# lzzcd001/MeshDiffusion

Measured on AMD Instinct MI355X. Metric: denoise steps/sec on 64^3x4 DMTet grids (sample-steps/s = n_gpus*batch*steps/wall), higher is better.
Workload: dtype f16f6 in the Winograd convs behind a GroupNorm (fp16 hi*hi MFMA + MX block-scaled e2m3 cross terms in a K-concatenated scaled MFMA at twice the e4m3 rate; operands and weights equalised per input channel by a power of two: md_wino_equaliser, after the load-time calibration from the measured operand

## Files before the change

### include/meshdiffusion_hip.h

```cpp
#ifndef MESHDIFFUSION_HIP_H
#define MESHDIFFUSION_HIP_H

#include <stdint.h>

#ifdef __cplusplus
extern "C" {
#endif

#define MD_OK 0
#define MD_ERR_BAD_ARG (-1)
#define MD_ERR_UNSUPPORTED (-2)
#define MD_ERR_NO_DEVICE (-3)

#define MD_ABI_VERSION 16

enum {
  MD_CFG_C3_128 = 0,
  MD_CFG_C3_128_K16 = 1,
  MD_CFG_C3_32 = 2,
  MD_CFG_C3_LOW = 3,
  MD_CFG_C3_S2 = 4,
  MD_CFG_G1_128 = 5,
  MD_CFG_G1_128_LOW = 6,
  MD_CFG_G1_64_LOW = 7,
// ... 26 lines not shown
  float alpha;
  int32_t cfg;
  int32_t batch;
  int32_t rows;
  int32_t rows_alloc;
  int32_t kdim;
  int32_t D, H, W;
  int32_t ups;
  int32_t a_src;
  int32_t out_mode;
  int32_t a_rows;
  int64_t a_bstride;
  int64_t bias_bstride;
  int64_t res_bstride;
  int64_t b_bstride;
  float* partial;
  int32_t ksplit;
  int32_t prec;
  double* stats;
  int32_t stagger;
  int32_t b_mode;
  const void* b2;
  const float* b_ac;
  int64_t b2_bstride;
  int32_t b_split;
  int32_t b_silu;
} MdGemmConvArgs;

int md_abi_version(void);
int md_device_count(void);

int md_gemm_conv(const MdGemmConvArgs* args, void* stream);
int64_t md_gemm_conv_partial_bytes(const MdGemmConvArgs* args);
int md_gemm_conv_cfg_info(int32_t cfg, int32_t* nt, int32_t* kc, int32_t* cols,
                          int32_t* taps, int32_t* lds_bytes, int32_t* threads);

int md_pack_weights(const float* w, void* wpk, int32_t rows, int32_t kdim, int32_t taps,
                    int64_t s_row, int64_t s_k, int64_t s_tap, int32_t nt, int32_t kc,
                    int32_t prec, void* stream);
int64_t md_packed_weight_bytes(int32_t rows, int32_t kdim, int32_t taps, int32_t nt, int32_t kc);

int md_gn_stats(const float* x, double* sums, int32_t batch, int32_t C, int64_t P,
                int32_t c_total, int32_t c_off, void* stream);
int md_gn_finalize(const double* sums, const float* gamma, const float* beta,
                   float* params, int32_t batch, int32_t c_total, int32_t groups,
                   int64_t P, float eps, float* ac, void* stream);
int md_gn_apply(const float* x, const float* params, void* out, void* out_raw, int32_t batch,
                int32_t C, int64_t P, int32_t c_total, int32_t c_off, int32_t norm,
                int32_t silu, float drop_p, uint64_t drop_seed, void* stream);
int md_dropout_scale(float* out, int32_t batch, int32_t C, int64_t P, int32_t c_total, int32_t c_off,
                     float drop_p, uint64_t drop_seed, void* stream);
int md_zero(void* p, int64_t bytes, void* stream);

int md_timestep_embedding(const float* t, float* emb, int32_t batch, int32_t dim, void* stream);
int md_linear(const float* x, const float* w, const float* bias, float* y, int32_t batch,
              int32_t in_dim, int32_t out_dim, int32_t silu_in, void* stream);

int md_fold_dx(const float* y, const float* bias, float* out, int32_t batch, int32_t co, int32_t kx, int32_t rows_alloc,
               int32_t D, int32_t H, int32_t W, void* stream);
int md_ncdhw_to_s16b_xfold(const float* x, void* out, int32_t batch, int32_t C, int32_t kx, int32_t c_pad, int32_t D, int32_t H,
                           int32_t W, void* stream);
int md_ncdhw_to_s16b(const float* x, void* out, int32_t batch, int32_t C, int32_t c_pad,
                     int64_t P, void* stream);
int md_f32b_to_ncdhw(const float* x, float* out, int32_t batch, int32_t C, int64_t P, void* stream);
int md_ncdhw_to_f32b(const float* x, float* out, int32_t batch, int32_t C, int64_t P, void* stream);
int md_s16b_to_ncdhw(const void* x, float* out, int32_t batch, int32_t C, int64_t P, void* stream);
// ... 257 lines not shown
```

### meshdiffusion_amd/_lib.py

```python
import ctypes as C
import os

_HERE = os.path.dirname(os.path.abspath(__file__))
LIB_PATH = os.environ.get("MD_LIB") or os.path.join(_HERE, "libmeshdiffusion_hip.so")

(CFG_C3_128, CFG_C3_128_K16, CFG_C3_32, CFG_C3_LOW, CFG_C3_S2, CFG_G1_128, CFG_G1_128_LOW, CFG_G1_64_LOW,
 CFG_C3_128_V2, CFG_C3_128_SW, CFG_C3_128_PIPE) = range(11)
(CFG_C3_128_FAST, CFG_C5_128_K16, CFG_C5_32_K16, CFG_C3_128_W4, CFG_C3X_32, CFG_C5X_32_K16, CFG_C3X_128_K16, CFG_C5X_128,
 CFG_G1_128_N128) = range(14, 23)
OUT_F32B, OUT_S16B, OUT_NCDHW = 0, 1, 2
PREC_BF16X3, PREC_FP16X2 = 0, 1
A_PACKED, A_S16B = 0, 1
B_S16B, B_F32B_GN = 0, 1
CORRECTOR_LANGEVIN, CORRECTOR_ALD = 0, 1
SDE_REVERSE_DIFFUSION, SDE_EULER_MARUYAMA = 0, 1
LANGEVIN_SLABS = 64

CFG_NT_KC = {
    CFG_C3_128: (128, 32), CFG_C3_128_K16: (128, 16), CFG_C3_32: (32, 32), CFG_C3_LOW: (128, 32),
    CFG_C3_S2: (128, 32), CFG_G1_128: (128, 32), CFG_G1_128_LOW: (128, 32), CFG_G1_64_LOW: (64, 32),
    CFG_C3_128_V2: (128, 32), CFG_C3_128_SW: (128, 32), CFG_C3_128_PIPE: (128, 32),
    CFG_C3_128_FAST: (128, 32), CFG_C5_128_K16: (128, 16), CFG_C5_32_K16: (32, 16), CFG_C3_128_W4: (128, 32), CFG_C3X_32: (32, 32), CFG_C5X_32_K16: (32, 16), CFG_C3X_128_K16: (128, 16), CFG_C5X_128: (128, 32), CFG_G1_128_N128: (128, 32),
}
ABLATION_CFG_NT_KC = {c: (128, 32) for c in (101, 102, 103, 104, 105, 111, 113, 114, 116, 117, 118, 122)}


class MdGemmConvArgs(C.Structure):
    _fields_ = [
        ("a", C.c_void_p), ("b", C.c_void_p), ("out", C.c_void_p), ("bias", C.c_void_p),
        ("residual", C.c_void_p), ("alpha", C.c_float), ("cfg", C.c_int32), ("batch", C.c_int32),
        ("rows", C.c_int32), ("rows_alloc", C.c_int32), ("kdim", C.c_int32), ("D", C.c_int32),
        ("H", C.c_int32), ("W", C.c_int32), ("ups", C.c_int32), ("a_src", C.c_int32),
        ("out_mode", C.c_int32), ("a_rows", C.c_int32), ("a_bstride", C.c_int64),
        ("bias_bstride", C.c_int64), ("res_bstride", C.c_int64), ("b_bstride", C.c_int64), ("partial", C.c_void_p), ("ksplit", C.c_int32), ("prec", C.c_int32),
        ("stats", C.c_void_p), ("stagger", C.c_int32), ("b_mode", C.c_int32), ("b2", C.c_void_p), ("b_ac", C.c_void_p),
        ("b2_bstride", C.c_int64), ("b_split", C.c_int32), ("b_silu", C.c_int32),
    ]


class MdPackJob(C.Structure):
    _fields_ = [
        ("w", C.c_void_p), ("out", C.c_void_p), ("s_row", C.c_int64), ("s_k", C.c_int64), ("s_tap", C.c_int64),
        ("n_items", C.c_int64), ("block0", C.c_int64), ("rows", C.c_int32), ("kdim", C.c_int32), ("taps", C.c_int32),
        ("nt", C.c_int32), ("kc", C.c_int32), ("prec", C.c_int32), ("flip", C.c_int32), ("kind", C.c_int32),
    ]


PACK_WPK, PACK_WINO, PACK_WINO_F6 = 0, 1, 2
WINO_FMT = {False: 0, "f8": 1, "f6": 2}
ABI_VERSION = 16
_P, _I32, _I64, _F, _U64 = C.c_void_p, C.c_int32, C.c_int64, C.c_float, C.c_uint64

SIGNATURES = {
    "md_abi_version": (C.c_int, []),
    "md_device_count": (C.c_int, []),
    "md_gemm_conv": (C.c_int, [C.POINTER(MdGemmConvArgs), _P]),
    "md_gemm_conv_partial_bytes": (_I64, [C.POINTER(MdGemmConvArgs)]),
    "md_gemm_conv_cfg_info": (C.c_int, [_I32] + [C.POINTER(C.c_int32)] * 6),
    "md_pack_weights": (C.c_int, [_P, _P, _I32, _I32, _I32, _I64, _I64, _I64, _I32, _I32, _I32, _P]),
    "md_packed_weight_bytes": (_I64, [_I32, _I32, _I32, _I32, _I32]),
    "md_gn_stats": (C.c_int, [_P, _P, _I32, _I32, _I64, _I32, _I32, _P]),
    "md_gn_finalize": (C.c_int, [_P, _P, _P, _P, _I32, _I32, _I32, _I64, _F, _P, _P]),
    "md_gn_apply": (C.c_int, [_P, _P, _P, _P, _I32, _I32, _I64, _I32, _I32, _I32, _I32, _F, _U64, _P]),
    "md_dropout_scale": (C.c_int, [_P, _I32, _I32, _I64, _I32, _I32, _F, _U64, _P]),
    "md_zero": (C.c_int, [_P, _I64, _P]),
    "md_timestep_embedding": (C.c_int, [_P, _P, _I32, _I32, _P]),
    "md_linear": (C.c_int, [_P, _P, _P, _P, _I32, _I32, _I32, _I32, _P]),
    "md_ncdhw_to_s16b_xfold": (C.c_int, [_P, _P, _I32, _I32, _I32, _I32, _I32, _I32, _I32, _P]),
    "md_fold_dx": (C.c_int, [_P, _P, _P, _I32, _I32, _I32, _I32, _I32, _I32, _I32, _P]),
    "md_ncdhw_to_s16b": (C.c_int, [_P, _P, _I32, _I32, _I32, _I64, _P]),
    "md_f32b_to_ncdhw": (C.c_int, [_P, _P, _I32, _I32, _I64, _P]),
    "md_ncdhw_to_f32b": (C.c_int, [_P, _P, _I32, _I32, _I64, _P]),
    "md_s16b_to_ncdhw": (C.c_int, [_P, _P, _I32, _I32, _I64, _P]),
    "md_nin_f32": (C.c_int, [_P, _P, _I32, _I32, _P, _P, _P, _I32, _I32, _I64, _I32, _P]),
    "md_wino_operand_bytes": (_I64, [_I32, _I32, _I32, _I32, _I32]),
    "md_wino_prep": (C.c_int, [_P, _P, _I32, _I32, _P, _I32, _I32, _P, _I32, _I32, _I32, _I32, _F, _U64, _P]),
    "md_wino_weight_bytes": (_I64, [_I32, _I32]),
    "md_wino_pack_weights": (C.c_int, [_P, _P, _I32, _I32, _I64, _I64, _I32, _P]),
    "md_conv3_wino": (C.c_int, [_P, _P, _P, _P, _I64, _P, _I64, _P, _I32, _I32, _I32, _I32, _I32, _I32, _I32, _P]),
    "md_wino_equaliser": (C.c_int, [_P, _P, _P, _I32, _I32, _I64, _I64, _P, _P]),
    "md_wino_equaliser_measured": (C.c_int, [_P, _P, _P, _P, _I32, _I32, _I64, _I64, _P, _P]),
    "md_wino_operand_ms": (C.c_int, [_P, _P, _I32, _I32, _P, _I32, _I32, _I64, _P, _P]),
    "md_wino_prep_f8": (C.c_int, [_P, _P, _I32, _I32, _P, _I32, _I32, _P, _P, _I32, _I32, _I32, _I32, _P]),
    "md_wino_weight_bytes_f8": (_I64, [_I32, _I32]),
    "md_wino_pack_weights_f8": (C.c_int, [_P, _P, _P, _I32, _I32, _I64, _I64, _P]),
    "md_conv3_wino_f8": (C.c_int, [_P, _P, _P, _P, _I64, _P, _I64, _P, _I32, _I32, _I32, _I32, _I32, _I32, _P]),
    "md_absmax": (C.c_int, [_P, _I64, _P, _P]),
    "md_wino_prep_dual_f6": (C.c_int, [_P, _I32, _P, _P, _P, _F, _P, _I32, _I32, _I32, _I32, _P]),
    "md_conv3_wino_f6_scaled": (C.c_int, [_P, _P, _P, _P, _I64, _P, _I64, _P, _I32, _I32, _I32, _I32, _I32, _I32, _F, _P, _P]),
    "md_wino_prep_f6": (C.c_int, [_P, _P, _I32, _I32, _P, _I32, _I32, _P, _P, _I32, _I32, _I32, _I32, _P]),
# ... 139 lines not shown
```

### meshdiffusion_amd/build.py

```python
import os
import shutil
import subprocess
import sys

HERE = os.path.dirname(os.path.abspath(__file__))
CSRC = os.path.join(HERE, "csrc")
INCLUDE = os.path.join(os.path.dirname(HERE), "include")
_SUFFIX = os.environ.get("MD_LIB_SUFFIX", "")
OBJDIR = os.path.join(CSRC, "build" + _SUFFIX)
LIB_PATH = os.path.join(HERE, f"libmeshdiffusion_hip{_SUFFIX}.so")
ARCH = "gfx950"
SOURCES = ["capi.hip", "gemm_conv.hip", "conv3_main.hip", "conv3_wino.hip", "conv3_s2.hip", "conv3_head.hip", "conv3_stem.hip", "pack_batch.hip", "wino_prep2.hip", "wino_eq.hip", "norm.hip", "elementwise.hip", "sde_steps.hip", "attention.hip", "nin_stream.hip", "block_pass.hip", "train.hip", "backward.hip", "wgrad.hip", "wgrad_wino.hip", "dmtet.hip", "dmtet_bwd.hip", "pointcloud.hip", "raster.hip", "antialias.hip", "interp.hip", "fixedtopo.hip", "visibility.hip"]
FLAGS = ["-O3", "-std=c++17", "-fPIC", f"--offload-arch={ARCH}", f"-I{INCLUDE}", f"-I{CSRC}",
         "-munsafe-fp-atomics", "-Wno-unused-result"]


def _hipcc():
    exe = shutil.which("hipcc") or "/opt/rocm/bin/hipcc"
    if not os.path.exists(exe):
        raise RuntimeError("hipcc not found: cannot build libmeshdiffusion_hip.so")
    return exe


def _newer(target, deps):
    if not os.path.exists(target):
        return True
    t = os.path.getmtime(target)
    return any(os.path.getmtime(d) > t for d in deps)


def build(verbose=False, force=False):
    from concurrent.futures import ThreadPoolExecutor
    hipcc = _hipcc()
    os.makedirs(OBJDIR, exist_ok=True)
    headers = [os.path.join(CSRC, "md_common.h"), os.path.join(CSRC, "md_pack.h"), os.path.join(CSRC, "md_prep_f6.h"), os.path.join(CSRC, "md_raster_snap.h"), os.path.join(CSRC, "md_gather.h"), os.path.join(INCLUDE, "meshdiffusion_hip.h")]
    flags = FLAGS + (["-DMD_BUILD_ABLATIONS"] if os.environ.get("MD_BUILD_ABLATIONS") == "1" else [])
    flags = flags + os.environ.get("MD_EXTRA_DEFINES", "").split()
    stamp = os.path.join(OBJDIR, "flags.txt")
    if not os.path.exists(stamp) or open(stamp).read() != " ".join(flags):
        force = True
    objs, jobs = [], []
    for src in SOURCES:
        sp = os.path.join(CSRC, src)
        if not os.path.exists(sp):
            raise RuntimeError(f"missing source {sp}")
# ... 27 lines not shown
```

### meshdiffusion_amd/hip_ops.py

```python
import ctypes as C
import math
import os

import torch

from . import _lib
from ._lib import (A_PACKED, A_S16B, PREC_BF16X3, PREC_FP16X2, CFG_C3_128, CFG_C3_128_V2, CFG_C3_128_SW, CFG_C3_128_PIPE, CFG_C3_128_FAST, CFG_C5_128_K16, CFG_C5_32_K16, CFG_C3_128_W4, CFG_C3X_32, CFG_C5X_32_K16, CFG_C3X_128_K16, CFG_C5X_128, CFG_G1_128_N128, CFG_C3_128_K16, CFG_C3_32, CFG_C3_LOW, CFG_C3_S2,
                   CFG_G1_128, CFG_G1_128_LOW, CFG_G1_64_LOW, CFG_NT_KC, OUT_F32B, OUT_NCDHW, OUT_S16B,
                   MdGemmConvArgs, check)


CFG_ABL1, CFG_ABL2, CFG_ABL3, CFG_ABL4, CFG_ABL5 = 101, 102, 103, 104, 105
CFG_F1, CFG_F3, CFG_F4, CFG_F6, CFG_F7, CFG_F8 = 111, 113, 114, 116, 117, 118
CFG_FAST_EC = 122
CONV_STAGGER = int(os.environ.get("MD_CONV_STAGGER", "0"))
DEBUG_ACT_FP16 = 2 if os.environ.get("MD_DEBUG_ACT_FP16") == "1" else 0
_MODES = ("bf16x3", "fp16x2", "f16f8", "f16f6")
DEFAULT_PRECISION = os.environ.get("MD_PRECISION", "bf16x3")
FORCE_PRECISION = os.environ.get("MD_FORCE_PRECISION")
WINO_EQ = os.environ.get("MD_WINO_EQ", "1") == "1"
F8_RAW = os.environ.get("MD_F8_RAW", "0") == "1"


def _decode(mode):
# ... 236 lines not shown

def prewarm_packs():
    layers = list(_PACK_LAYERS)
    _PACK_LAYERS.clear()
    n = 0
    for layer in layers:
        used = layer.__dict__.pop("_md_used", None) or {}
        if not PACK_BATCH:
            continue
        cache = layer.__dict__.get("_md_cache") or {}
        for name, (params, builder) in used.items():
            old = cache.get(name)
            consumed = old is not None and getattr(old[1], "_data", None) is not None
            obj = layer._cached(name, params, builder, mark=False)
            if consumed and hasattr(obj, "request"):
                obj.request()
                n += 1
    flush_packs()
    return n


def pack_s16b_from_matrix(w_kp, device):
    lib = _lib.load()
    w = w_kp.detach().to(device=device, dtype=torch.float32).contiguous()
    K, P = w.shape
    out = s16b_empty(1, K, P, device)
    check(lib.md_ncdhw_to_s16b(_ptr(w), _ptr(out), 1, K, K, P, _stream()), "md_ncdhw_to_s16b")
    return out


def gemm_conv(*, cfg, a, b, out, batch, rows, rows_alloc, kdim, dims, bias=None, bias_bstride=0,
              residual=None, res_bstride=0, alpha=1.0, ups=0, a_src=A_PACKED, a_rows=0, a_bstride=0,
              b_bstride=None, out_mode=OUT_F32B, ksplit=1, prec=PREC_BF16X3, stats=None, stagger=None,
              b_f32=None):
    lib = _lib.load()
    D, H, W = dims
    args = MdGemmConvArgs()
    args.a, args.out = a.data_ptr(), out.data_ptr()
    if b_f32 is not None:
        parts = b_f32["parts"]
        assert 1 <= len(parts) <= 2 and sum(c for _, c in parts) == kdim and all(c % 8 == 0 for _, c in parts)
        pin = D * H * W // (8 if ups else 1)
        args.b, args.b_split = parts[0][0].data_ptr(), parts[0][1]
        b_bstride = parts[0][1] * pin
        if len(parts) == 2:
            args.b2, args.b2_bstride = parts[1][0].data_ptr(), parts[1][1] * pin
        ac = b_f32.get("ac")
        args.b_ac = ac.data_ptr() if ac is not None else None
        args.b_silu = 1 if b_f32.get("silu") else 0
        args.b_mode = _lib.B_F32B_GN
    else:
        args.b = b.data_ptr()
    args.bias = bias.data_ptr() if bias is not None else None
    args.residual = residual.data_ptr() if residual is not None else None
    args.alpha = alpha
    args.cfg, args.batch, args.rows, args.rows_alloc, args.kdim = cfg, batch, rows, rows_alloc, kdim
    args.D, args.H, args.W, args.ups = D, H, W, ups
    args.a_src, args.out_mode, args.a_rows = a_src, out_mode, a_rows
    args.a_bstride, args.bias_bstride, args.res_bstride = a_bstride, bias_bstride, res_bstride
    if b_bstride is None:
        pin = D * H * W
        if ups:
            pin //= 8
        elif cfg == CFG_C3_S2:
            pin *= 8
        b_bstride = (kdim // 8) * 2 * pin * 8
    args.b_bstride = b_bstride
    args.prec = prec
    args.stats = stats.data_ptr() if stats is not None else None
    args.stagger = CONV_STAGGER if stagger is None else int(stagger)
    part = None
    if ksplit > 1:
        if out_mode != OUT_F32B:
            raise ValueError("split-K supports F32B output only")
        args.ksplit = ksplit
        part = torch.empty((ksplit * batch * rows_alloc * D * H * W,), dtype=torch.float32, device=out.device)
        args.partial = part.data_ptr()
    if PROFILE is None:
        check(lib.md_gemm_conv(C.byref(args), _stream()), f"md_gemm_conv(cfg={cfg})")
    else:
        taps = _lib.cfg_info(cfg)["taps"]
        flops = 2.0 * batch * rows * kdim * taps * D * H * W
        pin = D * H * W // (8 if ups else 1) * (8 if cfg == CFG_C3_S2 else 1)
        abytes = 4.0 * (batch * kdim * pin + rows * kdim * taps + batch * rows * D * H * W * (2 if residual is not None else 1))
        e0, e1 = torch.cuda.Event(enable_timing=True), torch.cuda.Event(enable_timing=True)
        e0.record()
        check(lib.md_gemm_conv(C.byref(args), _stream()), f"md_gemm_conv(cfg={cfg})")
        e1.record()
        PROFILE.append((cfg, flops, e0, e1, abytes,
                        f"{kdim}->{rows}@{D}x{H}x{W}" + ("/ups" if ups else "") + (f"/ks{ksplit}" if ksplit > 1 else "") +
                        ("/res" if residual is not None else "") + ("/stats" if stats is not None else "")))
    return out


WINO = os.environ.get("MD_WINO", "1") == "1"
WINO_PREP_V2 = os.environ.get("MD_WINO_PREP_V2", "1") == "1"
WINO_TRAIN_FWD = os.environ.get("MD_WINO_TRAIN_FWD", "1") == "1"


class WinoWeight:

    def __init__(self, w, device, kind="conv"):
        lib = _lib.load()
        w = w.detach().to(device=device, dtype=torch.float32).contiguous()
        _require_cuda(w, "weight")
        assert w.dim() == 5 and tuple(w.shape[2:]) == (3, 3, 3)
        if kind == "conv":
            self.rows, self.kdim = w.shape[0], w.shape[1]
            s_row, s_k, flip = self.kdim * 27, 27, 0
        elif kind == "conv_dgrad":
            self.rows, self.kdim = w.shape[1], w.shape[0]
            s_row, s_k, flip = 27, self.rows * 27, 1
        else:
            raise ValueError(kind)
        nbytes = lib.md_wino_weight_bytes(self.rows, self.kdim)
        if nbytes <= 0:
            raise _lib.MeshDiffusionHipError("md_wino_weight_bytes: unsupported weight shape")
        self._data, self._queued = None, False
        self._src = dict(kind=_lib.PACK_WINO, w=w, w_off=0, nbytes=nbytes, rows=self.rows, kdim=self.kdim, taps=9, s_row=s_row,
                         s_k=s_k, s_tap=0, nt=0, kc=0, prec=PREC_BF16X3, flip=flip)

    def request(self):
# ... 670 lines not shown
    check(lib.md_ddim_step(_ptr(x64), _ptr(eps), _ptr(mask), _ptr(coef), _ptr(partial), _ptr(pmask), int(ch), _ptr(x_out),
                           _ptr(x0_out), _ptr(x_f32), B, Cc, P, _stream()), "md_ddim_step")
    return x_out, x0_out, x_f32


def inpaint_blend_(x, src, pmask, gmask, ch, src_bstride=0):
    lib = _lib.load()
    B, Cc = x.shape[0], x.shape[1]
    P = x[0, 0].numel()
    check(lib.md_inpaint_blend(_ptr(x), _ptr(src), _ptr(pmask), _ptr(gmask), B, Cc, ch, P, src_bstride,
                               _stream()), "md_inpaint_blend")
    return x


def inpaint_renoise_(x, x_mean, z, pmask, gmask, coef, ch):
    lib = _lib.load()
    B, Cc = x.shape[0], x.shape[1]
    P = x[0, 0].numel()
    check(lib.md_inpaint_renoise(_ptr(x), _ptr(x_mean), _ptr(z), _ptr(pmask), _ptr(gmask), _ptr(coef), B, Cc,
                                 ch, P, _stream()), "md_inpaint_renoise")
    return x


def ksplit_for(cfg, batch, rows, kdim, spatial_out):
    info = _lib.cfg_info(cfg)
    tiles = max(1, spatial_out ** 3 // info["cols"]) * batch * ((rows + info["nt"] - 1) // info["nt"])
    ncc = kdim // info["kc"]
    ks = 1
    while tiles * ks < 256 and ks * 2 <= ncc and ks < 32:
        ks *= 2
    return ks


def conv_cfg_for(spatial, stride=1):
    if stride == 2:
        return CFG_C3_S2
    return CFG_C3_128_FAST if spatial % 8 == 0 else CFG_C3_LOW


NIN_N128 = os.environ.get("MD_NIN_N128", "1") == "1"


def gemm_cfg_for(ncols, nrows, hbm_bound=False):
    if hbm_bound and NIN_N128 and ncols % 128 == 0 and ncols >= 32768:
        return CFG_G1_128_N128
    if ncols % 256 == 0:
        return CFG_G1_128
    return CFG_G1_128_LOW if nrows % 128 == 0 else CFG_G1_64_LOW


def attn_scale(channels):
    return float(int(channels) ** (-0.5))


__all__ = [n for n in dir() if not n.startswith("_")]
_ = math
```

### meshdiffusion_amd/lib/diffusion/models/layers.py

```python
import math

import numpy as np
import torch
import torch.nn as nn

from .... import hip_ops as ops


def variance_scaling(scale, mode, distribution, in_axis=1, out_axis=0, dtype=torch.float32, device="cpu"):
    def init(shape, dtype=dtype, device=device):
        receptive = np.prod(shape) / shape[in_axis] / shape[out_axis]
        fan_in, fan_out = shape[in_axis] * receptive, shape[out_axis] * receptive
        denom = {"fan_in": fan_in, "fan_out": fan_out, "fan_avg": (fan_in + fan_out) / 2}[mode]
        var = scale / denom
        if distribution == "normal":
            return torch.randn(*shape, dtype=dtype, device=device) * np.sqrt(var)
        if distribution == "uniform":
            return (torch.rand(*shape, dtype=dtype, device=device) * 2.0 - 1.0) * np.sqrt(3 * var)
        raise ValueError("invalid distribution for variance scaling initializer")

    return init


def default_init(scale=1.0):
# ... 117 lines not shown
        f8 = (not b_f32.get("wino_only")) and ops.wino_f8_ok(
            S_out, drop=b_f32.get("drop"), keep=bool(b_f32.get("keep")), parts=b_f32["parts"],
            normalised=b_f32.get("ac") is not None
            or (ops.WINO_EQ and hasattr(wino, "measured") and wino.measured() is not None))
        if f8 and owner is not None and wino.site in getattr(owner, "md_bf16x3_sites", ()):
            f8 = False
        compact = (not b_f32.get("wino_only")) and ops.prep_compact_ok(ups, S_out, S_out, S_out, drop=b_f32.get("drop"), keep=bool(b_f32.get("keep")))
        nin = b_f32.get("nin")
        if (nin is not None and f8 == "f6" and not compact and not ups and not b_f32.get("drop") and not b_f32.get("keep")
                and not b_f32.get("wino_only") and ops.block_pass_ok(b_f32["parts"], nin[0].rows, B, S_out, S_out, S_out)):
            t, b_f32["res_out"] = ops.wino_prep_nin(b_f32["parts"], b_f32.get("ac"), b_f32.get("silu"), B, S_out,
                                                    wino.eq() if hasattr(wino, "eq") else None, nin[0], nin[1])
        else:
            t = ops.wino_prep(b_f32["parts"], b_f32.get("ac"), b_f32.get("silu"), ups, B, S_out, drop=b_f32.get("drop"),
                              keep=bool(b_f32.get("keep")), f8=f8, eq=wino.eq() if f8 and hasattr(wino, "eq") else None, compact=compact)
        if b_f32.get("keep"):
            b_f32["t_out"] = t
        ops.conv3_wino(wino(f8) if f8 else wino(), t, B, S_out, bias=bias, bias_bstride=bias_bstride, residual=residual,
                       res_bstride=res_bstride or 0, stats=stats, out=out)
        if f8 and ops.AUDIT is not None:
            t3 = ops.wino_prep(b_f32["parts"], b_f32.get("ac"), b_f32.get("silu"), ups, B, S_out, compact=compact)
            ref = ops.conv3_wino(wino(), t3, B, S_out, bias=bias, bias_bstride=bias_bstride, residual=residual, res_bstride=res_bstride or 0)
            ops.AUDIT.append(dict(owner=getattr(wino, "owner", None), site=getattr(wino, "site", None), fmt=f8, cin=pw.kdim, cout=pw.rows,
                                  S=S_out, rel_l2=float((torch.linalg.vector_norm(out - ref, dtype=torch.float64)
                                                         / torch.linalg.vector_norm(ref, dtype=torch.float64).clamp_min(1e-300)).item())))
            del t3, ref
        if stats is not None:
            out._md_sums = stats
        elif hasattr(out, "_md_sums"):
            del out._md_sums
        return out
    if b_f32 is not None and b_f32.get("wino_only"):
        b_f32 = None
    ksplit = ops.ksplit_for(pw.cfg, B, pw.rows, pw.kdim, S_out) if out_mode == ops.OUT_F32B else 1
    stats = None
    if (want_stats and ops.FUSE_GN_STATS and ((pw.cfg == ops.CFG_C3_128_FAST and ksplit == 1)
                                              or (ksplit > 1 and ops.SPLITK_STATS and P <= 512 and B * rows_alloc >= 2048))
            and out_mode == ops.OUT_F32B and rows_alloc == pw.rows):
        stats = ops.stats_zeros(B, rows_alloc, dev)
    ops.gemm_conv(cfg=pw.cfg, a=pw.data, b=act_s16, out=out, batch=B, rows=pw.rows,
                  rows_alloc=rows_alloc, kdim=pw.kdim, dims=(S_out, S_out, S_out), bias=bias,
                  bias_bstride=bias_bstride, residual=residual, res_bstride=res_bstride or 0, ups=ups,
                  out_mode=out_mode, ksplit=ksplit, prec=pw.prec, stats=stats, b_f32=b_f32)
    if stats is not None:
        out._md_sums = stats
    elif hasattr(out, "_md_sums"):
        del out._md_sums
    return out


def run_gemm(pw, act_s16, B, P, *, bias=None, bias_bstride=0, residual=None, out=None, out_mode=ops.OUT_F32B,
             alpha=1.0, b_bstride=None, b_f32=None):
    rows_alloc = ((pw.rows + 7) // 8) * 8
    dev = act_s16.device if act_s16 is not None else b_f32["parts"][0][0].device
    if out is None:
        out = (ops.f32b_empty if out_mode == ops.OUT_F32B else ops.s16b_empty)(B, rows_alloc, P, dev)
    return ops.gemm_conv(cfg=pw.cfg, a=pw.data, b=act_s16, out=out, batch=B, rows=pw.rows,
                         rows_alloc=rows_alloc, kdim=pw.kdim, dims=(1, 1, P), bias=bias,
                         bias_bstride=bias_bstride, residual=residual,
                         res_bstride=rows_alloc * P if residual is not None else 0, alpha=alpha,
                         out_mode=out_mode, b_bstride=b_bstride, b_f32=b_f32)


class NIN(HipLayer):

    def __init__(self, in_dim, num_units, init_scale=0.1):
        super().__init__()
        self.W = nn.Parameter(default_init(scale=init_scale)((in_dim, num_units)), requires_grad=True)
        self.b = nn.Parameter(torch.zeros(num_units), requires_grad=True)

    def packed(self, P, hbm_bound=False):
        rows = self.W.shape[1]
        cfg = ops.gemm_cfg_for(P, rows, hbm_bound)
        return self._cached(f"w{cfg}", [self.W], lambda: ops.PackedWeight(self.W, "nin", cfg, self.W.device))

    def forward_s16(self, act_s16, B, P, residual=None, out_mode=ops.OUT_F32B):
        return run_gemm(self.packed(P), act_s16, B, P, bias=self.b, residual=residual, out_mode=out_mode)

    def forward(self, x):
        parts, B, P, spatial = _parts_of(x)
        act = ops.gn_apply(parts, None, B, P, norm=False, silu=False)
        return ops.f32b_to_ncdhw(self.forward_s16(act, B, P), spatial)


class AttnBlock(HipLayer):

    def __init__(self, channels):
        super().__init__()
        self.GroupNorm_0 = nn.GroupNorm(num_groups=32, num_channels=channels, eps=1e-6)
        self.NIN_0 = NIN(channels, channels)
        self.NIN_1 = NIN(channels, channels)
        self.NIN_2 = NIN(channels, channels)
        self.NIN_3 = NIN(channels, channels, init_scale=0.0)
        self.channels = channels
# ... 278 lines not shown
```

Baseline: 114.1.

## Add split-K small-spatial conv kernel for low-resolution 3x3x3 and NIN layers

Adds a new HIP kernel for convolutions and 1x1 GEMMs at tiny spatial sizes (4^3 and 8^3). It stages the whole halo in LDS, double-buffers weights and activations, and splits the K dimension across many workgroups, targeting roughly 256 groups in total. It also adds a finishing kernel that reduces the split-K partials and computes the GroupNorm statistics in the same pass. The aim is to fill the GPU on low-resolution layers that the existing configs launch with too few tiles, at the cost of extra partial-buffer traffic and a reduction pass.

```diff
diff --git a/include/meshdiffusion_hip.h b/include/meshdiffusion_hip.h
--- a/include/meshdiffusion_hip.h
+++ b/include/meshdiffusion_hip.h
@@ -82,6 +82,7 @@
 
 int md_gemm_conv(const MdGemmConvArgs* args, void* stream);
 int64_t md_gemm_conv_partial_bytes(const MdGemmConvArgs* args);
+int md_small_conv(const MdGemmConvArgs* args, int32_t taps, void* stream);
 int md_gemm_conv_cfg_info(int32_t cfg, int32_t* nt, int32_t* kc, int32_t* cols,
                           int32_t* taps, int32_t* lds_bytes, int32_t* threads);
 
diff --git a/meshdiffusion_amd/_lib.py b/meshdiffusion_amd/_lib.py
--- a/meshdiffusion_amd/_lib.py
+++ b/meshdiffusion_amd/_lib.py
@@ -56,6 +56,7 @@
     "md_device_count": (C.c_int, []),
     "md_gemm_conv": (C.c_int, [C.POINTER(MdGemmConvArgs), _P]),
     "md_gemm_conv_partial_bytes": (_I64, [C.POINTER(MdGemmConvArgs)]),
+    "md_small_conv": (C.c_int, [C.POINTER(MdGemmConvArgs), _I32, _P]),
     "md_gemm_conv_cfg_info": (C.c_int, [_I32] + [C.POINTER(C.c_int32)] * 6),
     "md_pack_weights": (C.c_int, [_P, _P, _I32, _I32, _I32, _I64, _I64, _I64, _I32, _I32, _I32, _P]),
     "md_packed_weight_bytes": (_I64, [_I32, _I32, _I32, _I32, _I32]),
diff --git a/meshdiffusion_amd/build.py b/meshdiffusion_amd/build.py
--- a/meshdiffusion_amd/build.py
+++ b/meshdiffusion_amd/build.py
@@ -10,7 +10,7 @@
 OBJDIR = os.path.join(CSRC, "build" + _SUFFIX)
 LIB_PATH = os.path.join(HERE, f"libmeshdiffusion_hip{_SUFFIX}.so")
 ARCH = "gfx950"
-SOURCES = ["capi.hip", "gemm_conv.hip", "conv3_main.hip", "conv3_wino.hip", "conv3_s2.hip", "conv3_head.hip", "conv3_stem.hip", "pack_batch.hip", "wino_prep2.hip", "wino_eq.hip", "norm.hip", "elementwise.hip", "sde_steps.hip", "attention.hip", "nin_stream.hip", "block_pass.hip", "train.hip", "backward.hip", "wgrad.hip", "wgrad_wino.hip", "dmtet.hip", "dmtet_bwd.hip", "pointcloud.hip", "raster.hip", "antialias.hip", "interp.hip", "fixedtopo.hip", "visibility.hip"]
+SOURCES = ["capi.hip", "gemm_conv.hip", "small_conv.hip", "conv3_main.hip", "conv3_wino.hip", "conv3_s2.hip", "conv3_head.hip", "conv3_stem.hip", "pack_batch.hip", "wino_prep2.hip", "wino_eq.hip", "norm.hip", "elementwise.hip", "sde_steps.hip", "attention.hip", "nin_stream.hip", "block_pass.hip", "train.hip", "backward.hip", "wgrad.hip", "wgrad_wino.hip", "dmtet.hip", "dmtet_bwd.hip", "pointcloud.hip", "raster.hip", "antialias.hip", "interp.hip", "fixedtopo.hip", "visibility.hip"]
 FLAGS = ["-O3", "-std=c++17", "-fPIC", f"--offload-arch={ARCH}", f"-I{INCLUDE}", f"-I{CSRC}",
          "-munsafe-fp-atomics", "-Wno-unused-result"]
 
diff --git a/meshdiffusion_amd/csrc/small_conv.hip b/meshdiffusion_amd/csrc/small_conv.hip
--- /dev/null
+++ b/meshdiffusion_amd/csrc/small_conv.hip
@@ -0,0 +1,393 @@
+#include "md_common.h"
+
+namespace {
+#ifndef MD_SC_RM
+#define MD_SC_RM 1
+#endif
+constexpr int SC_NT = 128, SC_CT = 128, SC_KC = 32, SC_KG = SC_KC / 8;
+constexpr int SC_RM = MD_SC_RM, SC_THREADS = 64 * (SC_NT / (32 * SC_RM)) * 2;
+constexpr int SC_W_ITEMS = SC_KG * 2 * SC_NT;
+constexpr int SC_WPT = SC_W_ITEMS / SC_THREADS;
+constexpr int SC_HS = 288;
+constexpr int SC_ZERO = SC_HS - 1;
+constexpr int SC_A_ITEMS = SC_KG * 2 * SC_HS;
+constexpr int SC_LDS_ITEMS = 2 * SC_W_ITEMS + 2 * SC_A_ITEMS;
+static_assert(SC_LDS_ITEMS * 16 <= 160 * 1024, "LDS budget");
+}
+
+int md_launch_splitk_reduce(const MdGemmConvArgs& a, hipStream_t stream);
+
+template <int TAPS>
+__global__ __launch_bounds__(SC_THREADS) void md_small_conv_kernel(const MdGemmConvArgs A) {
+  constexpr int A_MAX = SC_KG * 2 * (TAPS == 1 ? SC_CT : SC_ZERO);
+  constexpr int AR_S16 = (A_MAX + SC_THREADS - 1) / SC_THREADS;
+  constexpr int AR = 2 * ((A_MAX / 2 + SC_THREADS - 1) / SC_THREADS);
+  static_assert(AR >= AR_S16, "activation registers cover the largest tile");
+  __shared__ __attribute__((aligned(16))) uint4 smem[SC_LDS_ITEMS];
+  uint4* wl = smem;
+  uint4* al = smem + 2 * SC_W_ITEMS;
+
+  const int tid = threadIdx.x;
+  const int lane = tid & 63, wid = tid >> 6;
+  const int wr = wid >> 1, wc = wid & 1;
+  const int j = lane & 31, h = lane >> 5;
+
+  const int H = A.H, W = A.W, D = A.D;
+  const int HW = H * W;
+  const int P = D * HW;
+  const int ncols = A.batch * P;
+  const int nct = (ncols + SC_CT - 1) / SC_CT;
+  const int nrt = (A.rows + SC_NT - 1) / SC_NT;
+  const int ksplit = A.ksplit > 1 ? A.ksplit : 1;
+  int ct, grp;
+  {
+    const int L = blockIdx.x, G = nrt * ksplit;
+    if ((G & 7) == 0) { const int q = L >> 3; ct = q % nct; grp = (q / nct) * 8 + (L & 7); }
+    else { ct = L % nct; grp = L / nct; }
+  }
+  const int rt = grp % nrt, kz = grp / nrt;
+  const int c0 = ct * SC_CT;
+  const int halo = (TAPS > 1) ? HW + W + 1 : 0;
+  const int NS = SC_CT + 2 * halo;
+  const int lo = c0 - halo;
+
+  const int ncc_total = A.kdim / SC_KC;
+  const int nsteps_total = ncc_total * TAPS;
+  const int s_lo = (int)(((int64_t)kz * nsteps_total) / ksplit);
+  const int s_hi = (int)(((int64_t)(kz + 1) * nsteps_total) / ksplit);
+  const int n = s_hi - s_lo;
+
+  const bool bf = A.b_mode == MD_B_F32B_GN;
+  const uint4* aptr = (const uint4*)A.a + (int64_t)rt * ncc_total * TAPS * SC_W_ITEMS;
+
+  if (tid < 2 * SC_KG * 2) al[tid * SC_HS + SC_ZERO] = make_uint4(0, 0, 0, 0);
+
+  int a_row[SC_RM];
+#pragma unroll
+  for (int rm = 0; rm < SC_RM; ++rm) a_row[rm] = (wr * SC_RM + rm) * 32 + j;
+  int lc[2], cb_[2], cp_[2], cz[2], cy[2], cx[2];
+  bool cvalid[2];
+#pragma unroll
+  for (int cm = 0; cm < 2; ++cm) {
+    lc[cm] = (wc * 2 + cm) * 32 + j;
+    const int col = c0 + lc[cm];
+    cvalid[cm] = col < ncols;
+    cb_[cm] = col / P;
+    cp_[cm] = col % P;
+    cx[cm] = cp_[cm] % W; cy[cm] = (cp_[cm] / W) % H; cz[cm] = cp_[cm] / HW;
+  }
+
+  f32x16 acc[SC_RM][2];
+#pragma unroll
+  for (int rm = 0; rm < SC_RM; ++rm)
+#pragma unroll
+    for (int cm = 0; cm < 2; ++cm)
+#pragma unroll
+      for (int r = 0; r < 16; ++r) acc[rm][cm][r] = 0.f;
+
+  auto w_issue = [&](uint4 (&wq)[SC_WPT], int s) __attribute__((always_inline)) {
+#pragma unroll
+    for (int i = 0; i < SC_WPT; ++i) { const uint4 v = aptr[(int64_t)s * SC_W_ITEMS + tid + i * SC_THREADS]; wq[i] = make_uint4(v.x, v.y, v.z, v.w); }
+  };
+  auto w_commit = [&](uint4 (&wq)[SC_WPT], int buf) __attribute__((always_inline)) {
+#pragma unroll
+    for (int i = 0; i < SC_WPT; ++i) wl[buf * SC_W_ITEMS + tid + i * SC_THREADS] = make_uint4(wq[i].x, wq[i].y, wq[i].z, wq[i].w);
+  };
+
+  const uint4* bptr = (const uint4*)A.b;
+  const uint4* bf_p1 = (const uint4*)A.b;
+  const uint4* bf_p2 = (const uint4*)A.b2;
+  const int split8 = A.b_split >> 3;
+  auto act_issue = [&](uint4 (&hr)[AR], unsigned& live, int cc) __attribute__((always_inline)) {
+    live = 0;
+    if (bf) {
+#pragma unroll
+      for (int i = 0; i < AR / 2; ++i) {
+        const int q = tid + i * SC_THREADS;
+        const int kg = q / NS, sl = q - kg * NS;
+        const int f = lo + sl;
+        uint4 v0 = make_uint4(0, 0, 0, 0), v1 = v0;
+        if (kg < SC_KG && f >= 0 && f < ncols) {
+          const int b = f / P, p = f - b * P;
+          const int g8 = cc * SC_KG + kg;
+          const uint4* cb = (g8 < split8) ? bf_p1 + (int64_t)b * (A.b_bstride / 4) + (int64_t)g8 * P * 2
+                                          : bf_p2 + (int64_t)b * (A.b2_bstride / 4) + (int64_t)(g8 - split8) * P * 2;
+          v0 = cb[(int64_t)p * 2]; v1 = cb[(int64_t)p * 2 + 1];
+          live |= 1u << i;
+        }
+        hr[2 * i] = v0; hr[2 * i + 1] = v1;
+      }
+    } else {
+#pragma unroll
+      for (int i = 0; i < AR_S16; ++i) {
+        const int item = tid + i * SC_THREADS;
+        const int gp = item / NS, sl = item - gp * NS;
+        const int f = lo + sl;
+        uint4 v = make_uint4(0, 0, 0, 0);
+        if (gp < SC_KG * 2 && f >= 0 && f < ncols) {
+          const int b = f / P, p = f - b * P;
+          v = bptr[(int64_t)b * (A.b_bstride / 8) + ((int64_t)((cc * SC_KG + (gp >> 1)) * 2 + (gp & 1))) * P + p];
+        }
+        hr[i] = v;
+      }
+    }
+  };
+  auto act_commit = [&](uint4 (&hr)[AR], unsigned live, int cc, int abuf) __attribute__((always_inline)) {
+    uint4* ab = al + abuf * SC_A_ITEMS;
+    if (bf) {
+#pragma unroll
+      for (int i = 0; i < AR / 2; ++i) {
+        const int q = tid + i * SC_THREADS;
+        const int kg = q / NS, sl = q - kg * NS;
+        if (kg >= SC_KG) continue;
+        const uint4 r0 = hr[2 * i], r1 = hr[2 * i + 1];
+        const float v[8] = {__uint_as_float(r0.x), __uint_as_float(r0.y), __uint_as_float(r0.z), __uint_as_float(r0.w),
+                            __uint_as_float(r1.x), __uint_as_float(r1.y), __uint_as_float(r1.z), __uint_as_float(r1.w)};
+        const bool lv = (live >> i) & 1u;
+        float yv[8];
+        if (A.b_ac != nullptr && lv) {
+          const int b = (lo + sl) / P;
+          const f32x4* ap = (const f32x4*)(A.b_ac + ((int64_t)b * A.kdim + (int64_t)(cc * SC_KG + kg) * 8) * 2);
+#pragma unroll
+          for (int e2 = 0; e2 < 4; ++e2) {
+            const f32x4 ac = ap[e2];
+#pragma unroll
+            for (int u = 0; u < 2; ++u) {
+              float y = v[2 * e2 + u] * ac[2 * u] + ac[2 * u + 1];
+              if (A.b_silu) y = y * __builtin_amdgcn_rcpf(1.0f + __builtin_amdgcn_exp2f(y * -1.4426950408889634f));
+              yv[2 * e2 + u] = y;
+            }
+          }
+        } else {
+#pragma unroll
+          for (int e = 0; e < 8; ++e) yv[e] = lv ? v[e] : 0.f;
+        }
+        uint32_t hi[4], lw[4];
+#pragma unroll
+        for (int e = 0; e < 4; ++e) md_split2(yv[2 * e], yv[2 * e + 1], hi[e], lw[e]);
+        ab[(kg * 2) * SC_HS + sl] = make_uint4(hi[0], hi[1], hi[2], hi[3]);
+        ab[(kg * 2 + 1) * SC_HS + sl] = make_uint4(lw[0], lw[1], lw[2], lw[3]);
+      }
+    } else {
+#pragma unroll
+      for (int i = 0; i < AR_S16; ++i) {
+        const int item = tid + i * SC_THREADS;
+        const int gp = item / NS, sl = item - gp * NS;
+        if (gp < SC_KG * 2) ab[gp * SC_HS + sl] = hr[i];
+      }
+    }
+  };
+
+  const bf16x8* wlf = (const bf16x8*)wl;
+  const bf16x8* alf = (const bf16x8*)al;
+
+  auto compute = [&](int wbuf, int abuf, int tap) __attribute__((always_inline)) {
+    const bf16x8* wb = wlf + wbuf * SC_W_ITEMS;
+    const bf16x8* ab = alf + abuf * SC_A_ITEMS;
+    int bs[2];
+#pragma unroll
+    for (int cm = 0; cm < 2; ++cm) {
+      if constexpr (TAPS > 1) {
+        const int dz = tap / 9, dy = (tap / 3) % 3, dx = tap % 3;
+        const int uz = cz[cm] + dz - 1, uy = cy[cm] + dy - 1, ux = cx[cm] + dx - 1;
+        const bool inb = cvalid[cm] & (uz >= 0) & (uz < D) & (uy >= 0) & (uy < H) & (ux >= 0) & (ux < W);
+        bs[cm] = inb ? lc[cm] + dz * HW + dy * W + dx : SC_ZERO;
+      } else {
+        bs[cm] = lc[cm];
+      }
+    }
+#pragma unroll
+    for (int ks = 0; ks < SC_KC / 16; ++ks) {
+      const int g = ks * 2 + h;
+      bf16x8 ahi[SC_RM], alo[SC_RM], bhi[2], blo[2];
+#pragma unroll
+      for (int rm = 0; rm < SC_RM; ++rm) {
+        ahi[rm] = wb[(g * 2 + 0) * SC_NT + a_row[rm]];
+        alo[rm] = wb[(g * 2 + 1) * SC_NT + a_row[rm]];
+      }
+#pragma unroll
+      for (int cm = 0; cm < 2; ++cm) {
+        bhi[cm] = ab[(g * 2 + 0) * SC_HS + bs[cm]];
+        blo[cm] = ab[(g * 2 + 1) * SC_HS + bs[cm]];
+      }
+#pragma unroll
+      for (int rm = 0; rm < SC_RM; ++rm)
+#pragma unroll
+        for (int cm = 0; cm < 2; ++cm) {
+          acc[rm][cm] = __builtin_amdgcn_mfma_f32_32x32x16_bf16(alo[rm], bhi[cm], acc[rm][cm], 0, 0, 0);
+          acc[rm][cm] = __builtin_amdgcn_mfma_f32_32x32x16_bf16(ahi[rm], blo[cm], acc[rm][cm], 0, 0, 0);
+          acc[rm][cm] = __builtin_amdgcn_mfma_f32_32x32x16_bf16(ahi[rm], bhi[cm], acc[rm][cm], 0, 0, 0);
+        }
+    }
+  };
+
+  uint4 wq0[SC_WPT], wq1[SC_WPT];
+  uint4 hq0[AR], hq1[AR];
+  unsigned live0 = 0, live1 = 0;
+  if constexpr (TAPS == 1) {
+    w_issue(wq0, s_lo); act_issue(hq0, live0, s_lo);
+    w_commit(wq0, 0); act_commit(hq0, live0, s_lo, 0);
+    if (n > 1) { w_issue(wq1, s_lo + 1); act_issue(hq1, live1, s_lo + 1); }
+    if (n > 2) { w_issue(wq0, s_lo + 2); act_issue(hq0, live0, s_lo + 2); }
+  } else {
+    w_issue(wq0, s_lo); act_issue(hq0, live0, s_lo / TAPS);
+    w_commit(wq0, 0); act_commit(hq0, live0, s_lo / TAPS, (s_lo / TAPS) & 1);
+    if (n > 1) w_issue(wq1, s_lo + 1);
+    if (n > 2) w_issue(wq0, s_lo + 2);
+  }
+  __syncthreads();
+  bool act_pending = false;
+  auto step = [&](int i, uint4 (&wn)[SC_WPT], uint4 (&hn)[AR], unsigned& liven) __attribute__((always_inline)) {
+    const int s = s_lo + i;
+    if (i + 1 < n) w_commit(wn, (i + 1) & 1);
+    if constexpr (TAPS == 1) {
+      if (i + 1 < n) act_commit(hn, liven, s + 1, (i + 1) & 1);
+      if (i + 3 < n) { w_issue(wn, s + 3); act_issue(hn, liven, s + 3); }
+      compute(i & 1, i & 1, 0);
+    } else {
+      if (i + 3 < n) w_issue(wn, s + 3);
+      const int cc = s / TAPS, tap = s - cc * TAPS;
+      const bool more = (cc + 1) * TAPS < s_hi;
+      if (more && !act_pending && tap >= TAPS - 7) { act_issue(hq0, live0, cc + 1); act_pending = true; }
+      if (more && tap == TAPS - 1) { act_commit(hq0, live0, cc + 1, (cc + 1) & 1); act_pending = false; }
+      compute(i & 1, cc & 1, tap);
+    }
+    __syncthreads();
+  };
+  for (int i = 0; i < n; i += 2) {
+    step(i, wq1, hq1, live1);
+    if (i + 1 < n) step(i + 1, wq0, hq0, live0);
+  }
+
+  const int rows_alloc = A.rows_alloc, rga = rows_alloc / 8;
+  if (ksplit > 1) {
+#pragma unroll
+    for (int cm = 0; cm < 2; ++cm) {
+      if (!cvalid[cm]) continue;
+      float* part = A.partial + ((int64_t)kz * A.batch + cb_[cm]) * rga * (int64_t)P * 8;
+#pragma unroll
+      for (int rm = 0; rm < SC_RM; ++rm)
+#pragma unroll
+        for (int q = 0; q < 4; ++q) {
+          const int row = rt * SC_NT + (wr * SC_RM + rm) * 32 + 8 * q + 4 * h;
+          if (row >= rows_alloc) continue;
+          f32x4 o4 = {acc[rm][cm][q * 4 + 0], acc[rm][cm][q * 4 + 1], acc[rm][cm][q * 4 + 2], acc[rm][cm][q * 4 + 3]};
+          *(f32x4*)(part + ((int64_t)(row >> 3) * P + cp_[cm]) * 8 + (row & 7)) = o4;
+        }
+    }
+    return;
+  }
+  const float alpha = A.alpha;
+#pragma unroll
+  for (int cm = 0; cm < 2; ++cm) {
+    if (!cvalid[cm]) continue;
+    const int b = cb_[cm];
+#pragma unroll
+    for (int rm = 0; rm < SC_RM; ++rm)
+#pragma unroll
+      for (int q = 0; q < 4; ++q) {
+        const int row = rt * SC_NT + (wr * SC_RM + rm) * 32 + 8 * q + 4 * h;
+        if (row >= rows_alloc) continue;
+        float v[4];
+#pragma unroll
+        for (int e = 0; e < 4; ++e) {
+          float x = alpha * acc[rm][cm][q * 4 + e];
+          if (A.bias != nullptr && row + e < A.rows) x += A.bias[(int64_t)b * A.bias_bstride + row + e];
+          v[e] = x;
+        }
+        const int64_t in_b = ((int64_t)(row >> 3) * P + cp_[cm]) * 8 + (row & 7);
+        if (A.residual != nullptr) {
+          const f32x4 r4 = *(const f32x4*)(A.residual + (int64_t)b * A.res_bstride + in_b);
+          v[0] += r4[0]; v[1] += r4[1]; v[2] += r4[2]; v[3] += r4[3];
+        }
+        f32x4 o4 = {v[0], v[1], v[2], v[3]};
+        *(f32x4*)((float*)A.out + (int64_t)b * rga * P * 8 + in_b) = o4;
+      }
+  }
+}
+
+__global__ __launch_bounds__(256) void md_small_conv_finish_stats_kernel(const MdGemmConvArgs A, int64_t P) {
+  __shared__ double red[4][16];
+  const int rga = A.rows_alloc / 8;
+  const int cg = blockIdx.x % rga, b = blockIdx.x / rga;
+  const int64_t slab = ((int64_t)b * rga + cg) * P * 8;
+  const int64_t slice = (int64_t)A.batch * rga * P * 8;
+  const int row = cg * 8 + (threadIdx.x & 1) * 4;
+  f32x4 bias = {0.f, 0.f, 0.f, 0.f};
+  if (A.bias != nullptr) {
+#pragma unroll
+    for (int e = 0; e < 4; ++e) if (row + e < A.rows) bias[e] = A.bias[(int64_t)b * A.bias_bstride + row + e];
+  }
+  double s1[4] = {0., 0., 0., 0.}, s2[4] = {0., 0., 0., 0.};
+  for (int64_t i = threadIdx.x; i < P * 2; i += 256) {
+    const int64_t e0 = slab + i * 4;
+    f32x4 s = *(const f32x4*)(A.partial + e0);
+    for (int z = 1; z < A.ksplit; ++z) {
+      const f32x4 v = *(const f32x4*)(A.partial + (int64_t)z * slice + e0);
+      s[0] += v[0]; s[1] += v[1]; s[2] += v[2]; s[3] += v[3];
+    }
+    f32x4 o;
+#pragma unroll
+    for (int e = 0; e < 4; ++e) o[e] = A.alpha * s[e] + bias[e];
+    if (A.residual != nullptr) {
+      const f32x4 rv = *(const f32x4*)(A.residual + (int64_t)b * A.res_bstride + (int64_t)cg * P * 8 + i * 4);
+      o[0] += rv[0]; o[1] += rv[1]; o[2] += rv[2]; o[3] += rv[3];
+    }
+    *(f32x4*)((float*)A.out + e0) = o;
+#pragma unroll
+    for (int e = 0; e < 4; ++e) { const double d = (double)o[e]; s1[e] += d; s2[e] += d * d; }
+  }
+#pragma unroll
+  for (int e = 0; e < 4; ++e)
+#pragma unroll
+    for (int o = 2; o < 64; o <<= 1) { s1[e] += __shfl_xor(s1[e], o, 64); s2[e] += __shfl_xor(s2[e], o, 64); }
+  const int lane = threadIdx.x & 63, wv = threadIdx.x >> 6;
+  if (lane < 2) {
+#pragma unroll
+    for (int e = 0; e < 4; ++e) { red[wv][(lane * 4 + e) * 2] = s1[e]; red[wv][(lane * 4 + e) * 2 + 1] = s2[e]; }
+  }
+  __syncthreads();
+  if (threadIdx.x < 16) {
+    const double t = (red[0][threadIdx.x] + red[1][threadIdx.x]) + (red[2][threadIdx.x] + red[3][threadIdx.x]);
+    A.stats[((int64_t)b * A.rows_alloc + cg * 8) * 2 + threadIdx.x] += t;
+  }
+}
+
+template <int TAPS>
+static int sc_launch(const MdGemmConvArgs& a, hipStream_t stream) {
+  const int64_t P = (int64_t)a.D * a.H * a.W;
+  const int64_t ncols = (int64_t)a.batch * P;
+  const int nct = (int)((ncols + SC_CT - 1) / SC_CT), nrt = (a.rows + SC_NT - 1) / SC_NT;
+  const int ks = a.ksplit > 1 ? a.ksplit : 1;
+  MD_HIP_CLEAR_ERROR();
+  hipLaunchKernelGGL(md_small_conv_kernel<TAPS>, dim3((unsigned)(nct * nrt * ks)), dim3(SC_THREADS), 0, stream, a);
+  MD_HIP_CHECK_LAUNCH();
+  if (ks > 1 && a.stats != nullptr) {
+    hipLaunchKernelGGL(md_small_conv_finish_stats_kernel, dim3((unsigned)(a.batch * (a.rows_alloc / 8))), dim3(256), 0, stream, a, P);
+    MD_HIP_CHECK_LAUNCH();
+    return MD_OK;
+  }
+  if (ks > 1) return md_launch_splitk_reduce(a, stream);
+  return MD_OK;
+}
+
+extern "C" int md_small_conv(const MdGemmConvArgs* args, int32_t taps, void* stream) {
+  if (args == nullptr || args->a == nullptr || args->b == nullptr || args->out == nullptr) return MD_ERR_BAD_ARG;
+  const MdGemmConvArgs& a = *args;
+  if (taps != 1 && taps != 27) return MD_ERR_UNSUPPORTED;
+  if (a.kdim <= 0 || a.kdim % SC_KC != 0 || a.rows <= 0 || a.rows_alloc % 8 != 0 || a.rows_alloc < a.rows || a.batch <= 0) return MD_ERR_BAD_ARG;
+  if (a.D <= 0 || a.H <= 0 || a.W <= 0) return MD_ERR_BAD_ARG;
+  if (a.prec != MD_PREC_BF16X3 || a.a_src != MD_A_PACKED || a.out_mode != MD_OUT_F32B || a.ups) return MD_ERR_UNSUPPORTED;
+  const int64_t P = (int64_t)a.D * a.H * a.W;
+  if ((int64_t)a.batch * P > (1 << 30)) return MD_ERR_UNSUPPORTED;
+  if (taps == 27 && SC_CT + 2 * ((int64_t)a.H * a.W + a.W + 1) > SC_ZERO) return MD_ERR_UNSUPPORTED;
+  if (a.b_mode != MD_B_S16B) {
+    if (a.b_mode != MD_B_F32B_GN || (a.b_split & 7) || a.b_split <= 0 || (a.b_split < a.kdim && a.b2 == nullptr)) return MD_ERR_UNSUPPORTED;
+    if (a.b_silu && a.b_ac == nullptr) return MD_ERR_BAD_ARG;
+  }
+  const int ks = a.ksplit > 1 ? a.ksplit : 1;
+  if (ks > (a.kdim / SC_KC) * taps || (ks > 1 && a.partial == nullptr)) return MD_ERR_BAD_ARG;
+  if (a.stats != nullptr && ks <= 1) return MD_ERR_UNSUPPORTED;
+  hipStream_t st = (hipStream_t)stream;
+  return taps == 27 ? sc_launch<27>(a, st) : sc_launch<1>(a, st);
+}
diff --git a/meshdiffusion_amd/hip_ops.py b/meshdiffusion_amd/hip_ops.py
--- a/meshdiffusion_amd/hip_ops.py
+++ b/meshdiffusion_amd/hip_ops.py
@@ -292,7 +292,7 @@
 def gemm_conv(*, cfg, a, b, out, batch, rows, rows_alloc, kdim, dims, bias=None, bias_bstride=0,
               residual=None, res_bstride=0, alpha=1.0, ups=0, a_src=A_PACKED, a_rows=0, a_bstride=0,
               b_bstride=None, out_mode=OUT_F32B, ksplit=1, prec=PREC_BF16X3, stats=None, stagger=None,
-              b_f32=None):
+              b_f32=None, small_taps=0):
     lib = _lib.load()
     D, H, W = dims
     args = MdGemmConvArgs()
@@ -336,18 +336,24 @@
         args.ksplit = ksplit
         part = torch.empty((ksplit * batch * rows_alloc * D * H * W,), dtype=torch.float32, device=out.device)
         args.partial = part.data_ptr()
+    if small_taps:
+        def launch():
+            check(lib.md_small_conv(C.byref(args), small_taps, _stream()), f"md_small_conv(taps={small_taps})")
+    else:
+        def launch():
+            check(lib.md_gemm_conv(C.byref(args), _stream()), f"md_gemm_conv(cfg={cfg})")
     if PROFILE is None:
-        check(lib.md_gemm_conv(C.byref(args), _stream()), f"md_gemm_conv(cfg={cfg})")
+        launch()
     else:
-        taps = _lib.cfg_info(cfg)["taps"]
+        taps = small_taps or _lib.cfg_info(cfg)["taps"]
         flops = 2.0 * batch * rows * kdim * taps * D * H * W
         pin = D * H * W // (8 if ups else 1) * (8 if cfg == CFG_C3_S2 else 1)
         abytes = 4.0 * (batch * kdim * pin + rows * kdim * taps + batch * rows * D * H * W * (2 if residual is not None else 1))
         e0, e1 = torch.cuda.Event(enable_timing=True), torch.cuda.Event(enable_timing=True)
         e0.record()
-        check(lib.md_gemm_conv(C.byref(args), _stream()), f"md_gemm_conv(cfg={cfg})")
+        launch()
         e1.record()
-        PROFILE.append((cfg, flops, e0, e1, abytes,
+        PROFILE.append(("small" if small_taps else cfg, flops, e0, e1, abytes,
                         f"{kdim}->{rows}@{D}x{H}x{W}" + ("/ups" if ups else "") + (f"/ks{ksplit}" if ksplit > 1 else "") +
                         ("/res" if residual is not None else "") + ("/stats" if stats is not None else "")))
     return out
@@ -1084,6 +1090,39 @@
     return ks
 
 
+SMALL_CONV = os.environ.get("MD_SMALL_CONV", "1") == "1"
+SMALL_CONV_WGS = int(os.environ.get("MD_SMALL_CONV_WGS", "256"))
+SMALL_CONV_CLASSES = frozenset(os.environ.get("MD_SMALL_CONV_CLASSES", "c3_4,nin_64,nin_512").split(","))
+
+
+def small_conv_class(taps, kdim, P, dims):
+    if taps == 27:
+        D, H, W = dims
+        if 128 + 2 * (H * W + W + 1) > 287:
+            return None
+        return "c3_4" if P <= 64 else ("c3_8" if P <= 512 else None)
+    if taps == 1:
+        if P <= 64:
+            return "nin_64" if kdim >= 1024 else "nin_64s"
+        if P <= 512:
+            return "nin_512" if kdim >= 512 else "nin_512s"
+    return None
+
+
+def small_conv_ok(pw, taps, B, P, dims, out_mode=OUT_F32B, ups=0):
+    if not SMALL_CONV or ups or out_mode != OUT_F32B or pw.prec != PREC_BF16X3 or pw.kdim % 32:
+        return False
+    if pw.cfg not in ((CFG_C3_LOW, CFG_C3_128, CFG_C3_128_FAST) if taps == 27 else (CFG_G1_128, CFG_G1_128_LOW, CFG_G1_128_N128)):
+        return False
+    return small_conv_class(taps, pw.kdim, P, dims) in SMALL_CONV_CLASSES
+
+
+def small_conv_split(B, P, rows, kdim, taps):
+    tiles = ((B * P + 127) // 128) * ((rows + 127) // 128)
+    steps = (kdim // 32) * taps
+    return max(1, min(steps, 64, (SMALL_CONV_WGS + tiles // 2) // tiles))
+
+
 def conv_cfg_for(spatial, stride=1):
     if stride == 2:
         return CFG_C3_S2
diff --git a/meshdiffusion_amd/lib/diffusion/models/layers.py b/meshdiffusion_amd/lib/diffusion/models/layers.py
--- a/meshdiffusion_amd/lib/diffusion/models/layers.py
+++ b/meshdiffusion_amd/lib/diffusion/models/layers.py
@@ -173,7 +173,11 @@
         return out
     if b_f32 is not None and b_f32.get("wino_only"):
         b_f32 = None
-    ksplit = ops.ksplit_for(pw.cfg, B, pw.rows, pw.kdim, S_out) if out_mode == ops.OUT_F32B else 1
+    small = 27 if ops.small_conv_ok(pw, 27, B, P, (S_out, S_out, S_out), out_mode, ups) else 0
+    if small:
+        ksplit = ops.small_conv_split(B, P, pw.rows, pw.kdim, 27)
+    else:
+        ksplit = ops.ksplit_for(pw.cfg, B, pw.rows, pw.kdim, S_out) if out_mode == ops.OUT_F32B else 1
     stats = None
     if (want_stats and ops.FUSE_GN_STATS and ((pw.cfg == ops.CFG_C3_128_FAST and ksplit == 1)
                                               or (ksplit > 1 and ops.SPLITK_STATS and P <= 512 and B * rows_alloc >= 2048))
@@ -182,7 +186,7 @@
     ops.gemm_conv(cfg=pw.cfg, a=pw.data, b=act_s16, out=out, batch=B, rows=pw.rows,
                   rows_alloc=rows_alloc, kdim=pw.kdim, dims=(S_out, S_out, S_out), bias=bias,
                   bias_bstride=bias_bstride, residual=residual, res_bstride=res_bstride or 0, ups=ups,
-                  out_mode=out_mode, ksplit=ksplit, prec=pw.prec, stats=stats, b_f32=b_f32)
+                  out_mode=out_mode, ksplit=ksplit, prec=pw.prec, stats=stats, b_f32=b_f32, small_taps=small)
     if stats is not None:
         out._md_sums = stats
     elif hasattr(out, "_md_sums"):
@@ -196,11 +200,13 @@
     dev = act_s16.device if act_s16 is not None else b_f32["parts"][0][0].device
     if out is None:
         out = (ops.f32b_empty if out_mode == ops.OUT_F32B else ops.s16b_empty)(B, rows_alloc, P, dev)
+    small = 1 if b_bstride is None and ops.small_conv_ok(pw, 1, B, P, (1, 1, P), out_mode) else 0
     return ops.gemm_conv(cfg=pw.cfg, a=pw.data, b=act_s16, out=out, batch=B, rows=pw.rows,
                          rows_alloc=rows_alloc, kdim=pw.kdim, dims=(1, 1, P), bias=bias,
                          bias_bstride=bias_bstride, residual=residual,
                          res_bstride=rows_alloc * P if residual is not None else 0, alpha=alpha,
-                         out_mode=out_mode, b_bstride=b_bstride, b_f32=b_f32)
+                         out_mode=out_mode, b_bstride=b_bstride, b_f32=b_f32, small_taps=small,
+                         ksplit=ops.small_conv_split(B, P, pw.rows, pw.kdim, 1) if small else 1)
 
 
 class NIN(HipLayer):
```

Result: no change. 115.0 (median of 6 runs) (+0.7%).
